# bebop/poly

Measured on AMD Instinct MI355X. Metric: mash.Sketch k-mers hashed/s, higher is better.
Workload: dtype u32

## Files before the change

### poly_amd/csrc/mash_sketch.hip

```cpp
#include <hip/hip_runtime.h>

#include <algorithm>

#include "common.h"
#include "k1_tauq.h"
#include "host_pipeline.h"
#include "multi_device.h"
#include <memory>
#include <string>
#include <type_traits>
#include <vector>

#ifndef PH_WPE
#define PH_WPE 6
#endif
#ifndef PH_CAPK
#define PH_CAPK 12u
#endif
#ifndef PH_ABL
#define PH_ABL 0
#endif
#ifndef PH_SEL_ATOMIC
#define PH_SEL_ATOMIC 0
#endif
#ifndef PH_BS_WIN
#define PH_BS_WIN 4
#endif
static_assert(PH_BS_WIN == 0 || PH_BS_WIN == 4, "the rank pass takes four slots per thread: its window is four");
#ifndef PH_SLAB_SIG
#define PH_SLAB_SIG 6u
#endif
#ifndef PH_SLAB_CW
#define PH_SLAB_CW 6u
#endif
#ifndef PH_SLAB_CF
#define PH_SLAB_CF 0u
#endif
#ifndef PH_SLAB_WPE
#define PH_SLAB_WPE 8
#endif

namespace polyhip {
namespace k1 {

constexpr int THREADS = 256;
constexpr int WAVES = THREADS / 64;
#ifndef PH_WTW
#define PH_WTW 512
#endif
constexpr int WTW = PH_WTW;
constexpr int TW = WTW * WAVES;
constexpr int GROUPS = WTW / (4 * 64);
constexpr int NB = 2048;
constexpr uint32_t MARK0 = 0xFFFFFFFFu, MARK1 = 0u;
constexpr uint32_t LUT_DW = 256;
constexpr int GBATCH = 32;
constexpr uint32_t WL_POSITIONAL = 0x80000000u;
constexpr uint32_t C1 = 0xcc9e2d51u, C2 = 0x1b873593u;

__device__ __forceinline__ uint32_t rotl32(uint32_t x, int r) { return (x << r) | (x >> (32 - r)); }

__device__ __forceinline__ uint32_t premix(uint32_t k)
{
    k *= C1;
    k = rotl32(k, 15);
    k *= C2;
    return k;
}

__device__ __forceinline__ uint32_t chain(uint32_t h) { return rotl32(h, 13) * 5u + 0xe6546b64u; }

__device__ __forceinline__ uint32_t fmix32(uint32_t h)
{
    h ^= h >> 16;
    h *= 0x85ebca6bu;
    h ^= h >> 13;
    h *= 0xc2b2ae35u;
    h ^= h >> 16;
    return h;
}

__device__ __forceinline__ uint32_t funnel_bytes(uint32_t hi, uint32_t lo, uint32_t sh)
{
    return __builtin_amdgcn_alignbyte(hi, lo, sh);
}

__device__ __forceinline__ uint32_t wave_incl_scan(uint32_t v)
{
    v += (uint32_t)__builtin_amdgcn_update_dpp(0, (int)v, 0x111, 0xF, 0xF, true);
    v += (uint32_t)__builtin_amdgcn_update_dpp(0, (int)v, 0x112, 0xF, 0xF, true);
    v += (uint32_t)__builtin_amdgcn_update_dpp(0, (int)v, 0x114, 0xF, 0xF, true);
    v += (uint32_t)__builtin_amdgcn_update_dpp(0, (int)v, 0x118, 0xF, 0xF, true);
    v += (uint32_t)__builtin_amdgcn_update_dpp(0, (int)v, 0x142, 0xA, 0xF, false);
    v += (uint32_t)__builtin_amdgcn_update_dpp(0, (int)v, 0x143, 0xC, 0xF, false);
    return v;
}

struct Smem {
    uint32_t *seqb;
    uint32_t *P;
    uint32_t *cand;
    uint32_t *binned;
    uint32_t *misc;
    uint32_t *lut;
    uint32_t *bins;
    uint32_t *biglist;
    uint32_t listcap;
};

constexpr uint32_t BIG_BIN = 32;
constexpr uint32_t BIG_LIST_CAP = 512;

template <class Bin, class Emit>
__device__ __attribute__((noinline)) void rank_big_bins(const uint32_t *__restrict__ binned, const Bin *__restrict__ bins,
                                              const uint32_t *__restrict__ biglist, uint32_t nbig, uint32_t s, Emit emit)
{
    const int lane = threadIdx.x & 63, wave = threadIdx.x >> 6;
    const uint64_t below = (1ull << lane) - 1ull;
    for (uint32_t q = wave; q < nbig; q += WAVES) {
        const uint32_t b = biglist[q];
        const uint32_t st = b ? bins[b - 1] : 0u, en = bins[b];
        uint32_t base = st, lastv = 0;
        bool first = true;
        while (base < s && base < en) {
            uint32_t m = 0xFFFFFFFFu;
            bool has = false;
            for (uint32_t x = st + lane; x < en; x += 64) {
                const uint32_t o = binned[x];
                if (first || o > lastv) {
                    m = min(m, o);
                    has = true;
                }
            }
            if (__ballot(has) == 0ull)
                break;
#pragma unroll
            for (int d = 32; d >= 1; d >>= 1)
                m = min(m, (uint32_t)__shfl_xor((int)m, d, 64));
            for (uint32_t x0 = st; x0 < en; x0 += 64) {
                const uint32_t x = x0 + lane;
                const bool eq = x < en && binned[x] == m;
                const uint64_t mask = __ballot(eq);
                const uint32_t pos = base + (uint32_t)__builtin_popcountll(mask & below);
                if (eq && pos < s)
                    emit(pos, m);
                base += (uint32_t)__builtin_popcountll(mask);
            }
            lastv = m;
            first = false;
        }
    }
}

template <class ForEach>
__device__ uint32_t bottom_s(const Smem &sm, uint32_t s, uint32_t tau, uint32_t binned_cap, bool keep_partial,
                             ForEach for_each)
{
    const int tid = threadIdx.x;
    uint32_t *bins = sm.P;
    const int sig = 32 - __builtin_clz(tau | 1u);
    const int shift = sig > 11 ? sig - 11 : 0;
    __syncthreads();

    for (int b = tid; b < NB; b += THREADS)
        bins[b] = 0;
    if (tid == 0)
        sm.misc[8] = 0;
    __syncthreads();
    for_each([&](uint32_t h) {
        if (h <= tau)
            atomicAdd(&bins[h >> shift], 1u);
    });
    __syncthreads();

    {
        uint32_t v[8], sum = 0;
#pragma unroll
        for (int i = 0; i < 8; ++i) {
            v[i] = bins[8 * tid + i];
            sum += v[i];
        }
        uint32_t incl = sum;
#pragma unroll
        for (int d = 1; d < 64; d <<= 1) {
            uint32_t t = __shfl_up(incl, d, 64);
            if ((tid & 63) >= d)
                incl += t;
        }
        if ((tid & 63) == 63)
            sm.misc[4 + (tid >> 6)] = incl;
        __syncthreads();
        uint32_t run = incl - sum;
        for (int w = 0; w < (tid >> 6); ++w)
            run += sm.misc[4 + w];
#pragma unroll
        for (int i = 0; i < 8; ++i) {
            bins[8 * tid + i] = run;
            run += v[i];
            if (v[i] > BIG_BIN) {
                const uint32_t slot = atomicAdd(&sm.misc[8], 1u);
                if (slot < BIG_LIST_CAP)
                    sm.seqb[slot] = (uint32_t)(8 * tid + i);
            }
        }
// ... 178 lines not shown
#pragma unroll
            for (int c = 0; c < 4; ++c)
                h[c] ^= k;
        }
#pragma unroll
        for (int c = 0; c < 4; ++c)
            h[c] = PH_ABL == 3 ? h[c] : fmix32(h[c]);
        emit(4u * (uint32_t)wq, h);
    }
    wave_sync();
}

template <int KS, bool LOCKSTEP, class Before, class EmitFull, class EmitPart>
__device__ __forceinline__ void run_tiles(const Smem &sm, const uint32_t *__restrict__ gdw, uint32_t gsh,
                                          int64_t gbytes, int64_t nwin, uint32_t k, uint32_t n_seq_dw, uint32_t n_P_w,
                                          Before before, EmitFull emit_full, EmitPart emit_part)
{
    const int wave = threadIdx.x >> 6;
    uint32_t *seqb = sm.seqb + wave * n_seq_dw;
    uint32_t *P = sm.P + wave * n_P_w;
    const int64_t stage_bytes = (int64_t)n_seq_dw * 4 + 4;
    auto is_full = [&](int64_t t0) { return (nwin - t0) >= (int64_t)WTW && t0 + stage_bytes <= gbytes; };
    Stager<KS> st;
    const int64_t first = (int64_t)wave * WTW;
    if (first < nwin)
        st.load(gdw, gsh, gbytes, first, n_seq_dw, is_full(first));
    for (int64_t T0 = 0; T0 < nwin; T0 += TW) {
        if (LOCKSTEP)
            before(T0);
        const int64_t t0 = T0 + first;
        if (t0 >= nwin)
            continue;
        const bool full = is_full(t0);
        st.store(seqb, gdw, gsh, gbytes, t0, n_seq_dw, full);
        wave_sync();
        if (t0 + TW < nwin)
            st.load(gdw, gsh, gbytes, t0 + TW, n_seq_dw, is_full(t0 + TW));
        if (full) {
            tile_compute<KS>(seqb, P, sm.lut, k, [&](uint32_t w0, const uint32_t(&h)[4]) { emit_full(t0, w0, h, 4u); });
        } else {
            const uint32_t wl = (uint32_t)((nwin - t0) < (int64_t)WTW ? (nwin - t0) : (int64_t)WTW);
            tile_compute<KS>(seqb, P, sm.lut, k, [&](uint32_t w0, const uint32_t(&h)[4]) {
                emit_part(t0, w0, h, w0 >= wl ? 0u : (wl - w0 < 4u ? wl - w0 : 4u));
            });
        }
    }
}

__device__ __forceinline__ void append4(uint32_t *__restrict__ counter, uint32_t *__restrict__ cand, uint32_t cap,
                                        const uint32_t (&h)[4], uint32_t nvalid, uint32_t tau)
{
    bool a[4];
    uint64_t m[4];
    uint32_t cnt[4], total = 0;
#pragma unroll
    for (int c = 0; c < 4; ++c) {
        a[c] = (PH_ABL == 4 ? h[c] == 12345u : h[c] <= tau) && (uint32_t)c < nvalid;
        m[c] = __ballot(a[c]);
        cnt[c] = (uint32_t)__popcll(m[c]);
        total += cnt[c];
    }
    if (total == 0)
        return;
    uint32_t base = 0;
    if ((threadIdx.x & 63) == 0)
        base = atomicAdd(counter, total);
    base = __builtin_amdgcn_readfirstlane(base);
#pragma unroll
    for (int c = 0; c < 4; ++c) {
        if (a[c]) {
            const uint32_t idx = base + __builtin_amdgcn_mbcnt_hi((uint32_t)(m[c] >> 32),
                                                                  __builtin_amdgcn_mbcnt_lo((uint32_t)m[c], 0u));
            if (idx < cap)
                cand[idx] = h[c];
        }
        base += cnt[c];
    }
}

constexpr int BSU = 4;
constexpr int BS_R = 7;
constexpr int BS_R0 = 5;
constexpr uint32_t BS_MARGIN = (PH_BS_WIN + 3u) & ~3u;
static_assert(BS_MARGIN % 4u == 0 && LUT_DW % 4u == 0, "the rank pass reads binned by 16 bytes: binned[0] is 16-byte aligned");
#define BS_SYNC()              \
    do {                       \
        if (PH_ABL != 21)      \
            __syncthreads();   \
    } while (0)
typedef __attribute__((address_space(3))) uint32_t lds_u32;
__device__ __forceinline__ uint32_t lds_addr(const uint32_t *p)
{
    return (uint32_t)(uintptr_t)(const __attribute__((address_space(3))) uint32_t *)p;
}
__device__ __forceinline__ void lds_store4_masked(const uint32_t (&addr)[4], const uint32_t (&v)[4], const uint64_t (&mask)[4])
{
    uint64_t saved;
    asm volatile("s_mov_b64 %0, exec\n\t"
                 "s_mov_b64 exec, %9\n\t"
                 "ds_write_b32 %1, %5\n\t"
                 "s_mov_b64 exec, %10\n\t"
                 "ds_write_b32 %2, %6\n\t"
                 "s_mov_b64 exec, %11\n\t"
                 "ds_write_b32 %3, %7\n\t"
                 "s_mov_b64 exec, %12\n\t"
                 "ds_write_b32 %4, %8\n\t"
                 "s_mov_b64 exec, %0"
                 : "=&s"(saved)
                 : "v"(addr[0]), "v"(addr[1]), "v"(addr[2]), "v"(addr[3]), "v"(v[0]), "v"(v[1]), "v"(v[2]), "v"(v[3]),
                   "s"(mask[0]), "s"(mask[1]), "s"(mask[2]), "s"(mask[3])
                 : "memory");
}
__device__ __forceinline__ void lds_store_masked(uint32_t addr, uint32_t v, uint64_t mask)
{
    uint64_t saved;
    asm volatile("s_mov_b64 %0, exec\n\t"
                 "s_mov_b64 exec, %3\n\t"
                 "ds_write_b32 %1, %2\n\t"
                 "s_mov_b64 exec, %0"
                 : "=&s"(saved)
                 : "v"(addr), "v"(v), "s"(mask)
                 : "memory");
}

template <bool FIN, int BINS_AT = -1>
__device__ void bottom_s_fast(const Smem &sm, uint32_t s, uint32_t tau, uint32_t C, uint32_t nbf_log2,
                              uint32_t *__restrict__ outp, const uint32_t *__restrict__ src, uint32_t first,
                              uint32_t step, uint32_t cnt)
{
    const int tid = threadIdx.x;
    uint32_t tid_o = (uint32_t)tid;
    asm volatile("" : "+v"(tid_o));
    auto fin = [](uint32_t h) { return FIN ? h ^ (h >> 16) : h; };
    uint32_t *bins = sm.bins;
    const uint16_t *bins16 = reinterpret_cast<const uint16_t *>(bins);
    const int sig = 32 - __builtin_clz(tau | 1u);
    const int shift = sig > (int)nbf_log2 ? sig - (int)nbf_log2 : 0;
    auto one = [](uint32_t b) { return 1u << ((b & 1u) << 4); };
    const bool wide = nbf_log2 == 11u;
    uint32_t z;
    asm volatile("v_mov_b32 %0, 0" : "=v"(z));
    if (wide)
        reinterpret_cast<uint4 *>(bins)[tid_o] = make_uint4(z, z, z, z);
    else
        reinterpret_cast<uint2 *>(bins)[tid_o] = make_uint2(z, z);
    if (tid == 0)
        sm.misc[8] = 0;
    if (PH_BS_WIN) {
        if (tid < PH_BS_WIN)
            sm.binned[-1 - (int)tid_o] = 0u;
        else if (tid < 2 * PH_BS_WIN)
            sm.binned[C + tid_o - PH_BS_WIN] = 0xFFFFFFFFu;
    }
    const uint32_t ntrip = (cnt + step - 1u) / step;
    const bool regs = ntrip <= (uint32_t)BS_R && shift >= 1;
    const bool more = ntrip > (uint32_t)BS_R0;
    const uint32_t bins_at = BINS_AT >= 0 ? (uint32_t)BINS_AT : lds_addr(bins);
    uint32_t hr[BS_R], bin_at[BS_R], bin_inc[BS_R];
    uint32_t first_o = first;
    asm volatile("" : "+v"(first_o));
    auto reg_valid = [&](int u) { return first_o < (cnt > (uint32_t)u * step ? cnt - (uint32_t)u * step : 0u); };
    const uint32_t src_at = lds_addr(src) + 4u * first_o, last_at = lds_addr(src) + 4u * ((cnt ? cnt : 1u) - 1u);
    auto reg_load = [&](int u) {
        hr[u] = fin(*reinterpret_cast<const lds_u32 *>((uintptr_t)min(src_at + 4u * (uint32_t)u * step, last_at)));
    };
    auto reg_count = [&](int u) {
        const uint32_t a = hr[u] >> (shift - 1);
        const bool there = reg_valid(u);
        bin_at[u] = there ? a & ~3u : 4u * first_o;
        bin_inc[u] = there ? 1u << ((a & 2u) << 3) : 0u;
        asm volatile("" : "+v"(bin_at[u]), "+v"(bin_inc[u]));
        __hip_atomic_fetch_add(reinterpret_cast<lds_u32 *>((uintptr_t)(bin_at[u] + bins_at)), bin_inc[u], __ATOMIC_RELAXED,
                               __HIP_MEMORY_SCOPE_WORKGROUP);
    };
    if (regs) {
#pragma unroll
        for (int u = 0; u < BS_R0; ++u)
            reg_load(u);
#pragma unroll
        for (int u = BS_R0; u < BS_R; ++u)
            hr[u] = z;
        if (more) {
#pragma unroll
            for (int u = BS_R0; u < BS_R; ++u)
                reg_load(u);
        }
    }
    BS_SYNC();
    if (regs) {
#pragma unroll
        for (int u = 0; u < BS_R0; ++u)
            reg_count(u);
        if (more) {
#pragma unroll
            for (int u = BS_R0; u < BS_R; ++u)
                reg_count(u);
        }
    } else {
        for (uint32_t i0 = first; i0 < cnt; i0 += BSU * step) {
            uint32_t h[BSU];
#pragma unroll
            for (int u = 0; u < BSU; ++u)
                h[u] = i0 + u * step < cnt ? fin(src[i0 + u * step]) : 0u;
#pragma unroll
            for (int u = 0; u < BSU; ++u)
                if (i0 + u * step < cnt) {
                    const uint32_t b = h[u] >> shift;
                    atomicAdd(&bins[b >> 1], one(b));
                }
        }
    }
    BS_SYNC();
    {
        uint32_t w[4];
        if (wide) {
            const uint4 t = reinterpret_cast<const uint4 *>(bins)[tid_o];
            w[0] = t.x, w[1] = t.y, w[2] = t.z, w[3] = t.w;
        } else {
            const uint2 t = reinterpret_cast<const uint2 *>(bins)[tid_o];
            w[0] = t.x, w[1] = t.y, w[2] = 0u, w[3] = 0u;
        }
        uint32_t c[8], sum = 0;
#pragma unroll
        for (int i = 0; i < 8; ++i) {
            c[i] = (w[i >> 1] >> (16 * (i & 1))) & 0xFFFFu;
            sum += c[i];
        }
        const uint32_t incl = wave_incl_scan(sum);
        if ((tid & 63) == 63)
            sm.misc[4 + (tid >> 6)] = incl;
        BS_SYNC();
        uint32_t run = incl - sum;
        for (int w8 = 0; w8 < (tid >> 6); ++w8)
            run += sm.misc[4 + w8];
        const uint32_t b0 = tid_o << (wide ? 3 : 2);
#pragma unroll
        for (int i = 0; i < 4; ++i) {
            w[i] = run | ((run + c[2 * i]) << 16);
            run += c[2 * i] + c[2 * i + 1];
        }
        if (wide)
            reinterpret_cast<uint4 *>(bins)[tid_o] = make_uint4(w[0], w[1], w[2], w[3]);
        else
            reinterpret_cast<uint2 *>(bins)[tid_o] = make_uint2(w[0], w[1]);
        if (max(max(max(c[0], c[1]), max(c[2], c[3])), max(max(c[4], c[5]), max(c[6], c[7]))) > BIG_BIN) {
#pragma unroll
            for (int i = 0; i < 8; ++i)
                if (c[i] > BIG_BIN) {
                    const uint32_t slot = atomicAdd(&sm.misc[8], 1u);
                    if (slot < sm.listcap)
                        sm.biglist[slot] = b0 + (uint32_t)i;
                }
        }
    }
    BS_SYNC();
    if (regs) {
        uint32_t ret[BS_R];
        const uint32_t binned_at = __builtin_amdgcn_readfirstlane(lds_addr(sm.binned));
        auto reg_add = [&](int u) {
            ret[u] = __hip_atomic_fetch_add(reinterpret_cast<lds_u32 *>((uintptr_t)(bin_at[u] + bins_at)), bin_inc[u], __ATOMIC_RELAXED,
                                            __HIP_MEMORY_SCOPE_WORKGROUP);
        };
        auto reg_put = [&](int u) {
            const uint32_t at = __builtin_amdgcn_ubfe(ret[u], bin_inc[u] >> 12, 16u);
            lds_store_masked(binned_at + 4u * at, hr[u], __ballot(bin_inc[u] != 0u));
        };
#pragma unroll
        for (int u = 0; u < BS_R0; ++u)
            reg_add(u);
        if (more) {
#pragma unroll
            for (int u = BS_R0; u < BS_R; ++u)
                reg_add(u);
        }
#pragma unroll
        for (int u = 0; u < BS_R0; ++u)
            reg_put(u);
        if (more) {
#pragma unroll
            for (int u = BS_R0; u < BS_R; ++u)
                reg_put(u);
        }
        asm volatile("s_waitcnt lgkmcnt(0)" ::: "memory");
    } else {
        for (uint32_t i0 = first; i0 < cnt; i0 += BSU * step) {
            uint32_t h[BSU], at[BSU];
#pragma unroll
            for (int u = 0; u < BSU; ++u)
                h[u] = i0 + u * step < cnt ? fin(src[i0 + u * step]) : 0u;
#pragma unroll
            for (int u = 0; u < BSU; ++u)
                if (i0 + u * step < cnt) {
                    const uint32_t b = h[u] >> shift;
                    at[u] = (atomicAdd(&bins[b >> 1], one(b)) >> ((b & 1u) << 4)) & 0xFFFFu;
                }
#pragma unroll
            for (int u = 0; u < BSU; ++u)
                if (i0 + u * step < cnt)
                    sm.binned[at[u]] = h[u];
        }
    }
    BS_SYNC();
    const uint32_t nbig = sm.misc[8];
    const bool by_waves = nbig <= sm.listcap;
    auto rank_in_bin = [&](uint32_t j, uint32_t hv) {
        const uint32_t b = hv >> shift;
        const uint32_t start = b ? bins16[b - 1] : 0u, end = bins16[b];
        if (start >= s || (by_waves && end - start > BIG_BIN))
            return;
        uint32_t pos = start;
        for (uint32_t x = start; x < end; ++x) {
            const uint32_t o = sm.binned[x];
            pos += (o < hv) || (o == hv && x < j);
        }
        if (pos < s)
            outp[pos] = hv;
    };
    const uint32_t e_star = bins16[sm.binned[s - 1] >> shift];
#if PH_BS_WIN
    if (PH_ABL != 22) {
        const uint32_t lim = 1u << shift;
        auto put = [&](uint32_t pos, uint32_t hv) {
            *reinterpret_cast<uint32_t *>(reinterpret_cast<uint8_t *>(outp) + (pos << 2)) = hv;
        };
        for (uint32_t j = 4u * tid_o; j < e_star; j += 4u * THREADS) {
            const uint4 *__restrict__ w4 = reinterpret_cast<const uint4 *>(sm.binned + j);
            const uint4 q0 = w4[-1], q1 = w4[0], q2 = w4[1];
            const uint32_t v[12] = {q0.x, q0.y, q0.z, q0.w, q1.x, q1.y, q1.z, q1.w, q2.x, q2.y, q2.z, q2.w};
            const uint32_t n = e_star - j;
            uint32_t pos[4] = {j, j + 1u, j + 2u, j + 3u};
            bool far[4];
#pragma unroll
            for (int q = 0; q < 4; ++q) {
                const uint32_t hv = v[4 + q];
#pragma unroll
                for (int d = 0; d < 4; ++d) {
                    if (d > q - 1)
                        pos[q] -= v[3 + q - d] > hv ? 1u : 0u;
                    if (d > 2 - q)
                        pos[q] += v[5 + q + d] < hv ? 1u : 0u;
                }
                far[q] = ((v[q] ^ hv) < lim) | ((v[8 + q] ^ hv) < lim);
            }
#pragma unroll
            for (int a = 0; a < 4; ++a)
#pragma unroll
                for (int b = a + 1; b < 4; ++b) {
                    const uint32_t gt = v[4 + a] > v[4 + b] ? 1u : 0u;
                    pos[a] += gt;
                    pos[b] -= gt;
                }
#pragma unroll
            for (int q = 0; q < 4; ++q) {
                if (__builtin_expect(far[q], 0)) {
                    if ((uint32_t)q < n)
                        rank_in_bin(j + (uint32_t)q, v[4 + q]);
                } else if (pos[q] < s && (uint32_t)q < n) {
                    put(pos[q], v[4 + q]);
                }
            }
        }
    }
#else
    for (uint32_t j = tid; j < e_star; j += THREADS)
        rank_in_bin(j, sm.binned[j]);
#endif
    if (by_waves && nbig)
        rank_big_bins(sm.binned, bins16, sm.biglist, nbig, s, [outp](uint32_t pos, uint32_t hv) { outp[pos] = hv; });
}

struct ReadView {
    const uint32_t *gdw;
    uint32_t gsh;
    int64_t gbytes, nwin;
};

__device__ __forceinline__ ReadView view(const uint8_t *__restrict__ seqs, const uint64_t *__restrict__ offs,
                                         uint64_t r, uint32_t k)
{
    ReadView v;
    const uint64_t o0 = offs[r], o1 = offs[r + 1];
    const int64_t n = (int64_t)(o1 - o0);
    v.nwin = n - (int64_t)k;
    v.gsh = (uint32_t)((uintptr_t)(seqs + o0) & 3);
    v.gdw = reinterpret_cast<const uint32_t *>(seqs + o0 - v.gsh);
    v.gbytes = n + v.gsh;
    return v;
}

template <int KS>
__global__ __launch_bounds__(THREADS) __attribute__((amdgpu_waves_per_eu(PH_WPE, 8))) void sketch_fast_kernel(const uint8_t *__restrict__ seqs,
                                                             const uint64_t *__restrict__ offs, uint64_t nseq,
                                                             uint32_t k_rt, uint32_t s, uint32_t *__restrict__ out,
                                                             uint32_t n_seq_dw, uint32_t n_P_w, uint32_t n_P,
                                                             uint32_t capf, uint32_t nbf_log2)
{
    extern __shared__ __attribute__((aligned(16))) uint32_t smem_raw[];
    Smem sm;
    sm.seqb = smem_raw;
    sm.P = sm.seqb + WAVES * n_seq_dw;
    sm.cand = sm.P + n_P;
    sm.binned = sm.cand + capf + BS_MARGIN;
    sm.misc = sm.binned + capf + BS_MARGIN;
    sm.lut = sm.misc + 16;
    sm.bins = sm.P;
    sm.biglist = sm.seqb;
    sm.listcap = BIG_LIST_CAP;

    const uint32_t k = KS > 0 ? (uint32_t)KS : k_rt;
    const int tid = threadIdx.x;
    sm.lut[tid] = premix((uint32_t)tid) ^ k;
    auto nothing = [](int64_t) {};

    for (uint64_t r = blockIdx.x; r < nseq; r += gridDim.x) {
        const ReadView rv = view(seqs, offs, r, k);
        if (rv.nwin <= 0)
            continue;
        uint32_t *__restrict__ outp = out + r * (uint64_t)s;

        if (rv.nwin < (int64_t)s) {
            __syncthreads();
            auto put = [&](int64_t t0, uint32_t w0, const uint32_t(&h)[4], uint32_t nvalid) {
#pragma unroll
                for (int c = 0; c < 4; ++c)
                    if ((uint32_t)c < nvalid)
                        outp[t0 + w0 + c] = h[c];
            };
            run_tiles<KS, false>(sm, rv.gdw, rv.gsh, rv.gbytes, rv.nwin, k, n_seq_dw, n_P_w, nothing, put, put);
            continue;
        }

        uint32_t tau0 = 0xFFFFFFFFu;
        {
            const uint64_t target = (uint64_t)s + 6ull * (uint64_t)__builtin_sqrtf((float)s) + 16ull;
            if ((int64_t)target < rv.nwin)
                tau0 = (uint32_t)((target << 32) / (uint64_t)rv.nwin);
        }
        bool ok = tau0 != 0xFFFFFFFFu || rv.nwin <= (int64_t)capf;
        __syncthreads();
        if (tid == 0)
            sm.misc[0] = 0;
        __syncthreads();
        uint32_t C = 0;
        if (ok) {
            auto keep = [&](int64_t, uint32_t, const uint32_t(&h)[4], uint32_t nvalid) {
                append4(&sm.misc[0], sm.cand, capf, h, nvalid, tau0);
            };
            run_tiles<KS, false>(sm, rv.gdw, rv.gsh, rv.gbytes, rv.nwin, k, n_seq_dw, n_P_w, nothing, keep, keep);
            __syncthreads();
            C = sm.misc[0];
            ok = C >= s && C <= capf;
        }
        if (ok) {
            if (PH_ABL == 5) {
                for (uint32_t i = tid; i < s; i += THREADS)
                    outp[i] = sm.cand[i];
            } else {
                bottom_s_fast<false>(sm, s, tau0, C, nbf_log2, outp, sm.cand, (uint32_t)tid, THREADS, C);
            }
        } else if (tid == 0) {
            outp[0] = MARK0;
            outp[1] = MARK1;
        }
    }
}

template <int KS> struct Slabs {
    static constexpr int NBLK = KS >> 2, TAIL = KS & 3;
    static constexpr int DUPD = NBLK + 2;
    const uint32_t *__restrict__ gdw;
    uint32_t gsh;
    uint32_t *__restrict__ seqb;
    uint32_t *__restrict__ P;
    const uint32_t *__restrict__ lut;
    int lane;

    uint32_t u_inside;
    uint32_t gb32;
    template <bool SH> __device__ __forceinline__ void gload_inside(uint32_t u, uint32_t &lo, uint32_t &hi) const
    {
        const uint32_t *__restrict__ slab = gdw + (uint64_t)u * 64;
        uint32_t off = (uint32_t)lane * 4u;
        asm volatile("" : "+v"(off));
        const uint8_t *__restrict__ p = reinterpret_cast<const uint8_t *>(slab) + off;
        lo = *reinterpret_cast<const uint32_t *>(p);
        hi = SH ? *reinterpret_cast<const uint32_t *>(p + 4) : 0u;
    }
    __device__ __forceinline__ void gload(uint32_t u, uint32_t &lo, uint32_t &hi) const
    {
        const uint32_t *__restrict__ slab = gdw + (uint64_t)u * 64;
// ... 151 lines not shown
    S.u_inside = rv.gbytes >= 65 * 4 ? (uint32_t)(((rv.gbytes >> 2) - 65) >> 6) + 1u : 0u;
    S.gb32 = (uint32_t)rv.gbytes;
    const uint32_t nfull = (uint32_t)(rv.nwin >> 8), rem = (uint32_t)rv.nwin & 255u;
    uint32_t cnt = 0;
#if PH_SEL_ATOMIC
    capw -= 1u;
    if (S.lane == 0)
        seg[capw] = 0u;
#endif
    if (a >= b)
        return cnt;
    uint32_t l1, h1;
    S.gload(a, l1, h1);
    if (a & 1) {
        S.template stage<1>(l1, h1);
        wave_sync();
        S.gload(a + 1, l1, h1);
        S.template premix_unit<1>();
    } else {
        S.template stage<0>(l1, h1);
        wave_sync();
        S.gload(a + 1, l1, h1);
        S.template premix_unit<0>();
    }
    auto step = [&](auto par, auto main, auto sh, uint32_t i) {
        constexpr int P = decltype(par)::value;
        constexpr bool MAIN = decltype(main)::value, SH = decltype(sh)::value;
        uint32_t h[4];
        S.template stage<1 - P, SH>(l1, h1);
        wave_sync();
        if (MAIN)
            S.template gload_inside<SH>(i + 2, l1, h1);
        else
            S.gload(i + 2, l1, h1);
        if (PH_ABL != 15)
            S.template premix_unit<1 - P>();
        wave_sync();
        S.template hash<P>(h);
        if (PH_ABL == 11) {
            if ((h[0] ^ h[1] ^ h[2] ^ h[3]) == 0x12345u)
                seg[0] = h[0];
        } else if (MAIN || __builtin_expect(i < nfull, 1)) {
            append_own<false>(seg, capw, cnt, h, 4u, tauq);
        } else {
            const int mine = (int)rem - 4 * S.lane;
            append_own<true>(seg, capw, cnt, h, mine <= 0 ? 0u : (mine < 4 ? (uint32_t)mine : 4u), tauq);
        }
        wave_sync();
    };
    using P0 = std::integral_constant<int, 0>;
    using P1 = std::integral_constant<int, 1>;
    using T = std::true_type;
    using F = std::false_type;
    const uint32_t lim = nfull < b ? nfull : b;
    const uint32_t ins = S.u_inside >= 2u ? S.u_inside - 2u : 0u;
    const uint32_t m = ins < lim ? ins : lim;
    uint32_t i = a;
    auto main_loop = [&](auto sh) {
        if ((i & 1) && i < m)
            step(P1{}, T{}, sh, i++);
        for (; i + 1 < m; i += 2) {
            step(P0{}, T{}, sh, i);
            step(P1{}, T{}, sh, i + 1);
        }
        if (i < m)
            step(P0{}, T{}, sh, i++);
    };
    if (S.gsh)
        main_loop(T{});
    else
        main_loop(F{});
    for (; i < b; ++i) {
        if (i & 1)
            step(P1{}, F{}, T{}, i);
        else
            step(P0{}, F{}, T{}, i);
    }
    return cnt;
}

template <int KS>
__global__ __launch_bounds__(THREADS) __attribute__((amdgpu_waves_per_eu(PH_SLAB_WPE, 8))) void sketch_slab_kernel(
    const uint8_t *__restrict__ seqs, const uint64_t *__restrict__ offs, uint64_t nseq, uint32_t s, uint32_t *__restrict__ out,
    uint32_t n_seq_dw, uint32_t n_P_w, uint32_t n_span, uint32_t capw, uint32_t capf, uint32_t nbf_log2)
{
    extern __shared__ __attribute__((aligned(16))) uint32_t smem_raw[];
    Smem sm;
    sm.lut = smem_raw;
    sm.seqb = smem_raw + LUT_DW;
    sm.P = sm.seqb + WAVES * n_seq_dw;
    sm.bins = sm.seqb;
    sm.binned = sm.bins + ((1u << nbf_log2) >> 1) + BS_MARGIN;
    sm.biglist = sm.binned + capf + BS_MARGIN;
    sm.listcap = (uint32_t)(sm.seqb + n_span - sm.biglist);
    sm.misc = sm.seqb + n_span;
    sm.cand = sm.misc + 16;
    constexpr uint32_t k = (uint32_t)KS;
    const int tid = threadIdx.x, wave = __builtin_amdgcn_readfirstlane(tid >> 6);
    sm.lut[tid] = premix((uint32_t)tid) ^ k;
    uint32_t *seg = sm.cand + wave * capw;

    for (uint64_t r = blockIdx.x; r < nseq; r += gridDim.x) {
        const ReadView rv = view(seqs, offs, r, k);
        if (rv.nwin <= 0)
            continue;
        uint32_t *__restrict__ outp = out + r * (uint64_t)s;
        if (rv.nwin < (int64_t)s)
            continue;
        const uint32_t tauq = slab_tauq(s + PH_SLAB_SIG * (uint32_t)__builtin_sqrtf((float)s) + 16u, rv.nwin);
        __syncthreads();
        const uint32_t cw = PH_ABL == 14 ? tauq >> 31 : run_slabs<KS>(sm, rv, n_seq_dw, n_P_w, seg, capw, tauq);
        if ((tid & 63) == 0)
            sm.misc[10 + wave] = cw;
        __syncthreads();
        if (PH_ABL == 11 || PH_ABL == 12 || PH_ABL == 14) {
            if (sm.misc[10] + sm.misc[11] + sm.misc[12] + sm.misc[13] == 0xFFFFFFF0u)
                outp[0] = cw;
            continue;
        }
        const uint32_t c0 = sm.misc[10], c1 = sm.misc[11], c2 = sm.misc[12], c3 = sm.misc[13];
        const uint32_t C = c0 + c1 + c2 + c3;
        const bool ok = max(max(c0, c1), max(c2, c3)) <= capw - (PH_SEL_ATOMIC ? 1u : 0u) && C >= s && C <= capf;
        if (ok)
            bottom_s_fast<true, (int)(LUT_DW * 4u)>(sm, s, tauq, C, nbf_log2, outp, seg, (uint32_t)(tid & 63), 64u, cw);
        else if (tid == 0) {
            outp[0] = MARK0;
            outp[1] = MARK1;
        }
    }
}

template <int KS>
__global__ __launch_bounds__(THREADS) void sketch_general_kernel(const uint8_t *__restrict__ seqs,
                                                                const uint64_t *__restrict__ offs, uint32_t k_rt,
                                                                uint32_t s, uint32_t *__restrict__ out,
                                                                uint32_t n_seq_dw, uint32_t n_P_w, uint32_t n_P,
                                                                uint32_t cap, uint64_t nseq, int take_positional)
{
    extern __shared__ __attribute__((aligned(16))) uint32_t smem_raw[];
    Smem sm;
    sm.seqb = smem_raw;
    sm.P = sm.seqb + WAVES * n_seq_dw;
    sm.cand = sm.P + n_P;
    sm.binned = sm.cand + cap;
    sm.misc = sm.binned + cap;
    sm.lut = sm.misc + 16;
    __shared__ uint32_t wl[GBATCH];
    __shared__ uint32_t nwl;

    const uint32_t k = KS > 0 ? (uint32_t)KS : k_rt;
    const int tid = threadIdx.x;
    sm.lut[tid] = premix((uint32_t)tid) ^ k;

    for (uint64_t base = (uint64_t)blockIdx.x * GBATCH; base < nseq; base += (uint64_t)gridDim.x * GBATCH) {
        __syncthreads();
        if (tid == 0)
            nwl = 0;
        __syncthreads();
        {
            const uint64_t r = base + tid;
            if (tid < GBATCH && r < nseq) {
                const int64_t nwin = (int64_t)(offs[r + 1] - offs[r]) - (int64_t)k;
                uint32_t need = 0;
                if (nwin >= (int64_t)s) {
                    const uint32_t *row = out + r * (uint64_t)s;
                    if (row[0] == MARK0 && row[1] == MARK1)
                        need = 1;
                } else if (nwin > 0 && take_positional) {
                    need = 2;
                }
                if (need)
                    wl[atomicAdd(&nwl, 1u)] = (uint32_t)tid | (need == 2 ? WL_POSITIONAL : 0u);
            }
        }
        __syncthreads();
        const uint32_t nredo = nwl;
    for (uint32_t q = 0; q < nredo; ++q) {
        const uint32_t entry = wl[q];
        const uint64_t r = base + (entry & ~WL_POSITIONAL);
        const ReadView rv = view(seqs, offs, r, k);
        uint32_t *__restrict__ outp = out + r * (uint64_t)s;
        __syncthreads();
        if (entry & WL_POSITIONAL) {
            auto put = [&](int64_t t0, uint32_t w0, const uint32_t(&h)[4], uint32_t nvalid) {
#pragma unroll
                for (int c = 0; c < 4; ++c)
                    if ((uint32_t)c < nvalid)
                        outp[t0 + w0 + c] = h[c];
            };
            run_tiles<KS, false>(sm, rv.gdw, rv.gsh, rv.gbytes, rv.nwin, k, n_seq_dw, n_P_w, [](int64_t) {}, put, put);
            continue;
        }
        if (tid == 0) {
            sm.misc[0] = 0;
            sm.misc[1] = 0xFFFFFFFFu;
        }
        __syncthreads();
        auto shrink_shared = [&]() {
            const uint32_t C = sm.misc[0];
            bottom_s(sm, s, sm.misc[1], cap, true, [&](auto f) {
                for (uint32_t i = tid; i < C; i += THREADS)
                    f(sm.cand[i]);
            });
        };
        auto append = [&](int64_t, uint32_t, const uint32_t(&h)[4], uint32_t nvalid) {
            append4(&sm.misc[0], sm.cand, cap, h, nvalid, sm.misc[1]);
        };
// ... 89 lines not shown
#pragma unroll
            for (int c = 0; c < 4; ++c) {
                const int64_t w = base + c * THREADS + tid;
                if (w < nwin) {
                    const uint32_t h = murmur3_window(sp + w, k);
                    if (h <= tau)
                        sm.cand[atomicAdd(&misc[0], 1u)] = h;
                }
            }
        }
        __syncthreads();
        shrink();
        for (uint32_t i = tid; i < s; i += THREADS)
            outp[i] = sm.cand[i];
    }
}

__global__ __launch_bounds__(THREADS) void sketch_tiny_kernel(const uint8_t *__restrict__ seqs,
                                                             const uint64_t *__restrict__ offs, uint64_t nseq, uint32_t k,
                                                             uint32_t s, uint32_t *__restrict__ out,
                                                             unsigned long long *__restrict__ first_panic)
{
    const int tid = threadIdx.x;
    for (uint64_t r = blockIdx.x; r < nseq; r += gridDim.x) {
        const uint64_t o0 = offs[r];
        const int64_t nwin = (int64_t)(offs[r + 1] - o0) - (int64_t)k;
        if (nwin <= 0)
            continue;
        if (s == 0) {
            if (tid == 0)
                atomicMin(first_panic, (unsigned long long)r);
            continue;
        }
        const uint8_t *__restrict__ sp = seqs + o0;
        const uint32_t h0 = murmur3_window(sp, k);
        bool under = false;
        for (int64_t w = 1 + tid; w < nwin && !under; w += THREADS)
            under = murmur3_window(sp + w, k) < h0;
        if (__syncthreads_or(under ? 1 : 0)) {
            if (tid == 0)
                atomicMin(first_panic, (unsigned long long)r);
        } else if (tid == 0) {
            out[r] = h0;
        }
    }
}

struct Launch {
    uint32_t n_seq_dw, n_P_w, n_P, n_P_fast, nbf_log2, nbf_log2_slab, capf, cap, capw, capf_slab, n_span;
    size_t smem_fast, smem_general, smem_slab;
};

static Launch plan(uint32_t k, uint32_t s)
{
    Launch L;
    const uint32_t nblk = k / 4;
    L.n_seq_dw = ((WTW / 4 + nblk + 2) + 3u) & ~3u;
    L.n_P_w = WTW + 4 * nblk;
    L.n_P = WAVES * L.n_P_w;
    L.n_P_fast = L.n_P < 1024u ? 1024u : L.n_P;
    L.nbf_log2 = L.n_P_fast >= 2048u ? 11u : 10u;
    if (L.n_P < (uint32_t)NB)
        L.n_P = NB;
    const uint32_t s4 = (s + 3u) & ~3u;
    uint32_t rt = 1;
    while ((uint64_t)rt * rt < s)
        ++rt;
    L.capf = (s4 + PH_CAPK * rt + 64u + 63u) & ~63u;
    L.cap = s4 + TW + 64u;
    const size_t common = (size_t)WAVES * L.n_seq_dw + L.n_P + 16 + 256;
    L.smem_fast = ((size_t)WAVES * L.n_seq_dw + L.n_P_fast + 16 + 256 + 2 * (size_t)L.capf + 2 * BS_MARGIN) * 4;
    if (PH_ABL == 7)
        L.smem_fast = 70 * 1024;
    L.smem_general = (common + 2 * (size_t)L.cap) * 4;
    {
        const uint32_t target = s + PH_SLAB_SIG * rt + 16u;
        const uint32_t exp_w = (target + WAVES - 1) / WAVES;
        uint32_t rw = 1;
        while ((uint64_t)rw * rw < exp_w)
            ++rw;
        L.capw = (exp_w + PH_SLAB_CW * rw + 8u + 63u) & ~63u;
        L.capf_slab = PH_SLAB_CF ? ((target + PH_SLAB_CF * rt + 8u + 63u) & ~63u) : L.capf;
    }
    L.nbf_log2_slab = 11;
    {
        const uint32_t rings = WAVES * (L.n_seq_dw + L.n_P_w);
        const uint32_t sorted = ((1u << L.nbf_log2_slab) >> 1) + L.capf_slab + 2 * BS_MARGIN + L.capf_slab / (BIG_BIN + 1) + 1;
        L.n_span = rings > sorted ? rings : sorted;
    }
    L.smem_slab = ((size_t)LUT_DW + L.n_span + 16 + (size_t)WAVES * L.capw) * 4;
#ifdef PH_LDS_PAD
    L.smem_slab += PH_LDS_PAD;
#endif
    return L;
}

constexpr uint64_t SLAB_ROUNDS = 32;

static unsigned persistent_grid(size_t smem, uint64_t n, uint64_t rounds = 4)
{
    const uint64_t per_cu = std::max<uint64_t>(1, std::min<uint64_t>(8, (160 * 1024) / std::max<size_t>(smem, 1)));
    return (unsigned)std::min<uint64_t>(n, 256 * per_cu * rounds);
}

template <int KS>
static int launch(const uint8_t *d_seqs, const uint64_t *d_offs, uint64_t n, uint32_t k, uint32_t s,
                  uint32_t *d_out, const Launch &L, hipStream_t st)
{
    PH_REQUIRE(L.capf % 4u == 0 && L.capf_slab % 4u == 0 && (WAVES * L.n_seq_dw + L.n_P_fast + L.capf + BS_MARGIN) % 4u == 0 &&
                   (LUT_DW + ((1u << L.nbf_log2_slab) >> 1) + BS_MARGIN) % 4u == 0,
               "polyhip_mash_sketch_batch: the sorted buffer of the LDS layout is not 16-byte aligned");
    auto general = sketch_general_kernel<KS>;
    PH_HIP(hipFuncSetAttribute(reinterpret_cast<const void *>(general), hipFuncAttributeMaxDynamicSharedMemorySize,
                               (int)L.smem_general));
    bool slabs = false;
    if constexpr (KS > 0) {
        slabs = !env_is("POLYHIP_K1_SLABS", '0') && L.smem_slab <= 64 * 1024 && s < 32768u;
        if (slabs) {
            auto slab = sketch_slab_kernel<KS>;
            PH_HIP(hipFuncSetAttribute(reinterpret_cast<const void *>(slab), hipFuncAttributeMaxDynamicSharedMemorySize,
                                       (int)L.smem_slab));
            hipLaunchKernelGGL(slab, dim3(persistent_grid(L.smem_slab, n, SLAB_ROUNDS)), dim3(THREADS), L.smem_slab, st, d_seqs, d_offs, n, s,
                               d_out, L.n_seq_dw, L.n_P_w, L.n_span, L.capw, L.capf_slab, L.nbf_log2_slab);
        }
    }
    if (!slabs) {
        auto fast = sketch_fast_kernel<KS>;
        PH_HIP(hipFuncSetAttribute(reinterpret_cast<const void *>(fast), hipFuncAttributeMaxDynamicSharedMemorySize,
                                   (int)L.smem_fast));
        hipLaunchKernelGGL(fast, dim3(persistent_grid(L.smem_fast, n)), dim3(THREADS), L.smem_fast, st, d_seqs, d_offs, n,
                           k, s, d_out, L.n_seq_dw, L.n_P_w, L.n_P_fast, L.capf, L.nbf_log2);
    }
    PH_HIP(hipGetLastError());
    const unsigned ggrid = (unsigned)std::min<uint64_t>((n + GBATCH - 1) / GBATCH, persistent_grid(L.smem_general, n));
    hipLaunchKernelGGL(general, dim3(ggrid), dim3(THREADS), L.smem_general, st, d_seqs, d_offs, k, s, d_out, L.n_seq_dw,
                       L.n_P_w, L.n_P, L.cap, n, slabs ? 1 : 0);
    PH_HIP(hipGetLastError());
    return POLYHIP_OK;
}

}
}

using namespace polyhip;

extern "C" {

int polyhip_mash_sketch_batch_dev(const uint8_t *d_seqs, const uint64_t *d_offsets, uint64_t n, uint32_t k,
                                  uint32_t s, uint32_t *d_out, polyhip_stream_t stream)
{
    if (n == 0)
        return POLYHIP_OK;
    PH_REQUIRE(d_seqs && d_offsets && (d_out || s == 0), "polyhip_mash_sketch_batch: null pointer");
    PH_REQUIRE(s <= (1u << 24), "polyhip_mash_sketch_batch: SketchSize %u > 2^24 is not implemented", s);
    hipStream_t st = as_stream(stream);
    if (s < 2) {
        unsigned long long *d_first = nullptr, h_first = ~0ull;
        PH_HIP(hipMallocAsync(reinterpret_cast<void **>(&d_first), sizeof h_first, st));
        StreamFree guard{d_first, st};
        PH_HIP(hipMemsetAsync(d_first, 0xFF, sizeof h_first, st));
        hipLaunchKernelGGL(k1::sketch_tiny_kernel, dim3((unsigned)std::min<uint64_t>(n, 4096)), dim3(k1::THREADS), 0, st, d_seqs,
                           d_offsets, n, k, s, d_out, d_first);
        PH_HIP(hipGetLastError());
        PH_HIP(hipMemcpyAsync(&h_first, d_first, sizeof h_first, hipMemcpyDeviceToHost, st));
        PH_HIP(guard.release());
        PH_HIP(hipStreamSynchronize(st));
        if (h_first != ~0ull)
            return set_error(POLYHIP_ERR_PANIC,
                             "mash.Sketch with SketchSize %u indexes Sketches[-1] on sequence %llu (mash.go:%s): the reference panics",
                             s, h_first + (unsigned long long)md::base().item, s == 0 ? "96" : "98");
        return POLYHIP_OK;
    }
    const k1::Launch L = k1::plan(k <= 4096 ? k : 4096, s <= 8192 ? s : 8192);
    if (s > 8192 || k > 4096 || L.smem_general > 160 * 1024) {
        const uint32_t s4 = (s + 3u) & ~3u;
        const uint32_t cap = 2 * s4 + 2 * k1::WIDE_ROUND;
        const uint64_t per_wg = 2ull * cap * sizeof(uint32_t), budget = 4ull << 30;
        const unsigned grid = (unsigned)std::max<uint64_t>(
            1, std::min<uint64_t>(std::min<uint64_t>(n, s > 16384 ? 256 : 1024), budget / per_wg));
        uint32_t *scratch = nullptr;
        PH_HIP(hipMallocAsync(reinterpret_cast<void **>(&scratch), (size_t)grid * per_wg, st));
        StreamFree guard{scratch, st};
        hipLaunchKernelGGL(k1::sketch_wide_kernel, dim3(grid), dim3(k1::THREADS), 0, st, d_seqs, d_offsets, n, k, s, d_out, scratch,
                           cap);
        PH_HIP(hipGetLastError());
        PH_HIP(guard.release());
        return POLYHIP_OK;
    }
    const uint64_t CHUNK = 1ull << 30;
    for (uint64_t i0 = 0; i0 < n; i0 += CHUNK) {
        const uint64_t m = n - i0 < CHUNK ? n - i0 : CHUNK;
        const uint64_t *offs = d_offsets + i0;
        uint32_t *outp = d_out + i0 * (uint64_t)s;
        int rc;
        switch (k) {
        case 17: rc = k1::launch<17>(d_seqs, offs, m, k, s, outp, L, st); break;
        case 21: rc = k1::launch<21>(d_seqs, offs, m, k, s, outp, L, st); break;
        case 31: rc = k1::launch<31>(d_seqs, offs, m, k, s, outp, L, st); break;
        default: rc = k1::launch<0>(d_seqs, offs, m, k, s, outp, L, st); break;
        }
        if (rc != POLYHIP_OK)
            return rc;
    }
    return POLYHIP_OK;
}

// ... 157 lines not shown
```

Measured before the change: 999.1 billion.

## Pack bin-count scan, flag big bins via SWAR, add wave-level small-bin ranking

Reworks the bottom-s selection: the per-thread bin-count scan now works on packed 16-bit pairs with SWAR adds and perm instead of unpacking eight counters. Big bins are detected with a packed overflow test and stored as a 16-bit list (doubling list capacity). rank_big_bins makes its bin bounds wave-uniform and handles bins of at most 64 entries with a readlane comparison loop, and the per-element in-bin ranking moves into a separate noinline function. The slab kernel's bin count becomes a compile-time constant. This adds a 15-bit count limit, enforced by a new host check, plus extra code paths that could raise register pressure.

After: 1002 billion (median of 6 runs). Within noise of the previous version (+0.3%).

```diff
diff --git a/poly_amd/csrc/mash_sketch.hip b/poly_amd/csrc/mash_sketch.hip
--- a/poly_amd/csrc/mash_sketch.hip
+++ b/poly_amd/csrc/mash_sketch.hip
@@ -27,6 +27,12 @@
 #define PH_BS_WIN 4
 #endif
 static_assert(PH_BS_WIN == 0 || PH_BS_WIN == 4, "the rank pass takes four slots per thread: its window is four");
+#ifndef PH_BS_LIST_WIN
+#define PH_BS_LIST_WIN 0
+#endif
+#ifndef PH_BS_SCAN_PACKED
+#define PH_BS_SCAN_PACKED 1
+#endif
 #ifndef PH_SLAB_SIG
 #define PH_SLAB_SIG 6u
 #endif
@@ -111,15 +117,30 @@
 constexpr uint32_t BIG_BIN = 32;
 constexpr uint32_t BIG_LIST_CAP = 512;
 
-template <class Bin, class Emit>
+template <class Bin, class List, class Emit>
 __device__ __attribute__((noinline)) void rank_big_bins(const uint32_t *__restrict__ binned, const Bin *__restrict__ bins,
-                                              const uint32_t *__restrict__ biglist, uint32_t nbig, uint32_t s, Emit emit)
-{
-    const int lane = threadIdx.x & 63, wave = threadIdx.x >> 6;
+                                              const List *__restrict__ biglist, uint32_t nbig, uint32_t s, Emit emit)
+{
+    const int lane = threadIdx.x & 63, wave = __builtin_amdgcn_readfirstlane(threadIdx.x >> 6);
     const uint64_t below = (1ull << lane) - 1ull;
     for (uint32_t q = wave; q < nbig; q += WAVES) {
-        const uint32_t b = biglist[q];
-        const uint32_t st = b ? bins[b - 1] : 0u, en = bins[b];
+        const uint32_t b = __builtin_amdgcn_readfirstlane((uint32_t)biglist[q]);
+        const uint32_t st = b ? __builtin_amdgcn_readfirstlane((uint32_t)bins[b - 1]) : 0u;
+        const uint32_t en = __builtin_amdgcn_readfirstlane((uint32_t)bins[b]);
+        if (st >= s || en <= st)
+            continue;
+        if (en - st <= 64u) {
+            const uint32_t n = en - st;
+            const uint32_t mine = binned[st + min((uint32_t)lane, n - 1u)];
+            uint32_t pos = st;
+            for (uint32_t i = 0; i < n; ++i) {
+                const uint32_t o = (uint32_t)__builtin_amdgcn_readlane((int)mine, (int)i);
+                pos += (o < mine || (o == mine && i < (uint32_t)lane)) ? 1u : 0u;
+            }
+            if ((uint32_t)lane < n && pos < s)
+                emit(pos, mine);
+            continue;
+        }
         uint32_t base = st, lastv = 0;
         bool first = true;
         while (base < s && base < en) {
@@ -464,6 +485,8 @@
 constexpr int BS_R = 7;
 constexpr int BS_R0 = 5;
 constexpr uint32_t BS_MARGIN = (PH_BS_WIN + 3u) & ~3u;
+constexpr uint32_t NBF_LOG2_SLAB = 11;
+constexpr uint32_t BS_LIST_OVER = PH_BS_WIN && PH_BS_LIST_WIN ? (uint32_t)PH_BS_WIN : BIG_BIN;
 static_assert(BS_MARGIN % 4u == 0 && LUT_DW % 4u == 0, "the rank pass reads binned by 16 bytes: binned[0] is 16-byte aligned");
 #define BS_SYNC()              \
     do {                       \
@@ -505,14 +528,35 @@
                  : "memory");
 }
 
-template <bool FIN, int BINS_AT = -1>
-__device__ void bottom_s_fast(const Smem &sm, uint32_t s, uint32_t tau, uint32_t C, uint32_t nbf_log2,
+__device__ __attribute__((noinline)) void rank_whole_bins(const uint32_t *__restrict__ binned, const uint16_t *__restrict__ bins16,
+                                                          int shift, uint32_t s, uint32_t e_star, uint32_t skip_over,
+                                                          uint32_t *__restrict__ outp)
+{
+    for (uint32_t j = threadIdx.x; j < e_star; j += THREADS) {
+        const uint32_t hv = binned[j];
+        const uint32_t b = hv >> shift;
+        const uint32_t start = b ? bins16[b - 1] : 0u, end = bins16[b];
+        if (start >= s || end - start > skip_over)
+            continue;
+        uint32_t pos = start;
+        for (uint32_t x = start; x < end; ++x) {
+            const uint32_t o = binned[x];
+            pos += (o < hv) || (o == hv && x < j);
+        }
+        if (pos < s)
+            outp[pos] = hv;
+    }
+}
+
+template <bool FIN, int BINS_AT = -1, int NBF_LOG2 = 0>
+__device__ void bottom_s_fast(const Smem &sm, uint32_t s, uint32_t tau, uint32_t C, uint32_t nbf_log2_rt,
                               uint32_t *__restrict__ outp, const uint32_t *__restrict__ src, uint32_t first,
                               uint32_t step, uint32_t cnt)
 {
     const int tid = threadIdx.x;
     uint32_t tid_o = (uint32_t)tid;
     asm volatile("" : "+v"(tid_o));
+    const uint32_t nbf_log2 = NBF_LOG2 > 0 ? (uint32_t)NBF_LOG2 : nbf_log2_rt;
     auto fin = [](uint32_t h) { return FIN ? h ^ (h >> 16) : h; };
     uint32_t *bins = sm.bins;
     const uint16_t *bins16 = reinterpret_cast<const uint16_t *>(bins);
@@ -526,12 +570,12 @@
         reinterpret_cast<uint4 *>(bins)[tid_o] = make_uint4(z, z, z, z);
     else
         reinterpret_cast<uint2 *>(bins)[tid_o] = make_uint2(z, z);
-    if (tid == 0)
+    if (tid_o == 0u)
         sm.misc[8] = 0;
     if (PH_BS_WIN) {
-        if (tid < PH_BS_WIN)
+        if (tid_o < (uint32_t)PH_BS_WIN)
             sm.binned[-1 - (int)tid_o] = 0u;
-        else if (tid < 2 * PH_BS_WIN)
+        else if (tid_o < 2u * (uint32_t)PH_BS_WIN)
             sm.binned[C + tid_o - PH_BS_WIN] = 0xFFFFFFFFu;
     }
     const uint32_t ntrip = (cnt + step - 1u) / step;
@@ -602,38 +646,75 @@
             const uint2 t = reinterpret_cast<const uint2 *>(bins)[tid_o];
             w[0] = t.x, w[1] = t.y, w[2] = 0u, w[3] = 0u;
         }
-        uint32_t c[8], sum = 0;
+        const uint32_t b0 = tid_o << (wide ? 3 : 2);
+        constexpr uint32_t OVER = (0x7FFFu - BS_LIST_OVER) * 0x10001u;
+        const uint32_t f01 = ((w[0] + OVER) & 0x80008000u) | (((w[1] + OVER) & 0x80008000u) >> 1);
+        const uint32_t f23 = ((w[2] + OVER) & 0x80008000u) | (((w[3] + OVER) & 0x80008000u) >> 1);
+        const uint32_t flags = f01 | (f23 >> 2);
+        uint32_t run, sum;
+#if PH_BS_SCAN_PACKED
+        const uint32_t t = (w[0] + w[1]) + (w[2] + w[3]);
+        sum = (t & 0xFFFFu) + (t >> 16);
+#else
+        uint32_t c[8];
+        sum = 0;
 #pragma unroll
         for (int i = 0; i < 8; ++i) {
             c[i] = (w[i >> 1] >> (16 * (i & 1))) & 0xFFFFu;
             sum += c[i];
         }
+#endif
         const uint32_t incl = wave_incl_scan(sum);
-        if ((tid & 63) == 63)
-            sm.misc[4 + (tid >> 6)] = incl;
+        if ((tid_o & 63u) == 63u)
+            sm.misc[4 + (tid_o >> 6)] = incl;
+        if (__ballot(flags != 0u) != 0ull) {
+            const uint32_t nl = (uint32_t)__builtin_popcount(flags);
+            uint32_t slot = nl ? atomicAdd(&sm.misc[8], nl) : 0u;
+            uint16_t *list = reinterpret_cast<uint16_t *>(sm.biglist);
+#pragma unroll
+            for (int i = 0; i < 8; ++i)
+                if (flags & (1u << (16 * (i & 1) + 15 - (i >> 1)))) {
+                    if (slot < sm.listcap)
+                        list[slot] = (uint16_t)(b0 + (uint32_t)i);
+                    ++slot;
+                }
+        }
+        if (PH_BS_LIST_WIN && sig == 32 && tid_o == (uint32_t)(THREADS - 1)) {
+            const uint32_t top = (wide ? w[3] : w[1]) >> 16;
+            if (top != 0u && top <= BS_LIST_OVER) {
+                const uint32_t slot = atomicAdd(&sm.misc[8], 1u);
+                if (slot < sm.listcap)
+                    reinterpret_cast<uint16_t *>(sm.biglist)[slot] = (uint16_t)((1u << nbf_log2) - 1u);
+            }
+        }
         BS_SYNC();
-        uint32_t run = incl - sum;
-        for (int w8 = 0; w8 < (tid >> 6); ++w8)
+        run = incl - sum;
+#if PH_BS_SCAN_PACKED
+        {
+            const uint4 tot = *reinterpret_cast<const uint4 *>(sm.misc + 4);
+            const uint32_t wv = __builtin_amdgcn_readfirstlane(tid_o >> 6);
+            run += (tot.x & (wv > 0u ? ~0u : 0u)) + (tot.y & (wv > 1u ? ~0u : 0u)) + (tot.z & (wv > 2u ? ~0u : 0u));
+        }
+        uint32_t both = run | (run << 16);
+#pragma unroll
+        for (int i = 0; i < 4; ++i) {
+            const uint32_t cnts = w[i];
+            w[i] = both + (cnts << 16);
+            both = __builtin_amdgcn_perm(0u, w[i] + cnts, 0x03020302u);
+        }
+#else
+        for (int w8 = 0; w8 < (int)(tid_o >> 6); ++w8)
             run += sm.misc[4 + w8];
-        const uint32_t b0 = tid_o << (wide ? 3 : 2);
 #pragma unroll
         for (int i = 0; i < 4; ++i) {
             w[i] = run | ((run + c[2 * i]) << 16);
             run += c[2 * i] + c[2 * i + 1];
         }
+#endif
         if (wide)
             reinterpret_cast<uint4 *>(bins)[tid_o] = make_uint4(w[0], w[1], w[2], w[3]);
         else
             reinterpret_cast<uint2 *>(bins)[tid_o] = make_uint2(w[0], w[1]);
-        if (max(max(max(c[0], c[1]), max(c[2], c[3])), max(max(c[4], c[5]), max(c[6], c[7]))) > BIG_BIN) {
-#pragma unroll
-            for (int i = 0; i < 8; ++i)
-                if (c[i] > BIG_BIN) {
-                    const uint32_t slot = atomicAdd(&sm.misc[8], 1u);
-                    if (slot < sm.listcap)
-                        sm.biglist[slot] = b0 + (uint32_t)i;
-                }
-        }
     }
     BS_SYNC();
     if (regs) {
@@ -685,6 +766,7 @@
     BS_SYNC();
     const uint32_t nbig = sm.misc[8];
     const bool by_waves = nbig <= sm.listcap;
+#if !PH_BS_LIST_WIN
     auto rank_in_bin = [&](uint32_t j, uint32_t hv) {
         const uint32_t b = hv >> shift;
         const uint32_t start = b ? bins16[b - 1] : 0u, end = bins16[b];
@@ -698,6 +780,7 @@
         if (pos < s)
             outp[pos] = hv;
     };
+#endif
     const uint32_t e_star = bins16[sm.binned[s - 1] >> shift];
 #if PH_BS_WIN
     if (PH_ABL != 22) {
@@ -722,7 +805,7 @@
                     if (d > 2 - q)
                         pos[q] += v[5 + q + d] < hv ? 1u : 0u;
                 }
-                far[q] = ((v[q] ^ hv) < lim) | ((v[8 + q] ^ hv) < lim);
+                far[q] = (((v[q] ^ hv) < lim) & (j != 0u)) | ((v[8 + q] ^ hv) < lim);
             }
 #pragma unroll
             for (int a = 0; a < 4; ++a)
@@ -734,21 +817,31 @@
                 }
 #pragma unroll
             for (int q = 0; q < 4; ++q) {
+#if !PH_BS_LIST_WIN
                 if (__builtin_expect(far[q], 0)) {
                     if ((uint32_t)q < n)
                         rank_in_bin(j + (uint32_t)q, v[4 + q]);
-                } else if (pos[q] < s && (uint32_t)q < n) {
+                    continue;
+                }
+#endif
+                if (!far[q] && pos[q] < s && (uint32_t)q < n)
                     put(pos[q], v[4 + q]);
-                }
-            }
-        }
-    }
+            }
+        }
+    }
+    if (nbig == 0u)
+        return;
+    if (by_waves || !PH_BS_LIST_WIN)
+        rank_big_bins(sm.binned, bins16, reinterpret_cast<const uint16_t *>(sm.biglist), by_waves ? nbig : 0u, s,
+                      [outp](uint32_t pos, uint32_t hv) { outp[pos] = hv; });
+    else
+        rank_whole_bins(sm.binned, bins16, shift, s, e_star, 0xFFFFFFFFu, outp);
 #else
-    for (uint32_t j = tid; j < e_star; j += THREADS)
-        rank_in_bin(j, sm.binned[j]);
-#endif
+    rank_whole_bins(sm.binned, bins16, shift, s, e_star, by_waves ? BIG_BIN : 0xFFFFFFFFu, outp);
     if (by_waves && nbig)
-        rank_big_bins(sm.binned, bins16, sm.biglist, nbig, s, [outp](uint32_t pos, uint32_t hv) { outp[pos] = hv; });
+        rank_big_bins(sm.binned, bins16, reinterpret_cast<const uint16_t *>(sm.biglist), nbig, s,
+                      [outp](uint32_t pos, uint32_t hv) { outp[pos] = hv; });
+#endif
 }
 
 struct ReadView {
@@ -787,7 +880,7 @@
     sm.lut = sm.misc + 16;
     sm.bins = sm.P;
     sm.biglist = sm.seqb;
-    sm.listcap = BIG_LIST_CAP;
+    sm.listcap = 2u * BIG_LIST_CAP;
 
     const uint32_t k = KS > 0 ? (uint32_t)KS : k_rt;
     const int tid = threadIdx.x;
@@ -1105,7 +1198,7 @@
 template <int KS>
 __global__ __launch_bounds__(THREADS) __attribute__((amdgpu_waves_per_eu(PH_SLAB_WPE, 8))) void sketch_slab_kernel(
     const uint8_t *__restrict__ seqs, const uint64_t *__restrict__ offs, uint64_t nseq, uint32_t s, uint32_t *__restrict__ out,
-    uint32_t n_seq_dw, uint32_t n_P_w, uint32_t n_span, uint32_t capw, uint32_t capf, uint32_t nbf_log2)
+    uint32_t n_seq_dw, uint32_t n_P_w, uint32_t n_span, uint32_t capw, uint32_t capf)
 {
     extern __shared__ __attribute__((aligned(16))) uint32_t smem_raw[];
     Smem sm;
@@ -1113,15 +1206,17 @@
     sm.seqb = smem_raw + LUT_DW;
     sm.P = sm.seqb + WAVES * n_seq_dw;
     sm.bins = sm.seqb;
-    sm.binned = sm.bins + ((1u << nbf_log2) >> 1) + BS_MARGIN;
+    sm.binned = sm.bins + ((1u << NBF_LOG2_SLAB) >> 1) + BS_MARGIN;
     sm.biglist = sm.binned + capf + BS_MARGIN;
-    sm.listcap = (uint32_t)(sm.seqb + n_span - sm.biglist);
+    sm.listcap = 2u * (uint32_t)(sm.seqb + n_span - sm.biglist);
     sm.misc = sm.seqb + n_span;
     sm.cand = sm.misc + 16;
     constexpr uint32_t k = (uint32_t)KS;
     const int tid = threadIdx.x, wave = __builtin_amdgcn_readfirstlane(tid >> 6);
     sm.lut[tid] = premix((uint32_t)tid) ^ k;
     uint32_t *seg = sm.cand + wave * capw;
+    uint32_t capw_s = capw;
+    asm volatile("" : "+s"(capw_s));
 
     for (uint64_t r = blockIdx.x; r < nseq; r += gridDim.x) {
         const ReadView rv = view(seqs, offs, r, k);
@@ -1132,7 +1227,7 @@
             continue;
         const uint32_t tauq = slab_tauq(s + PH_SLAB_SIG * (uint32_t)__builtin_sqrtf((float)s) + 16u, rv.nwin);
         __syncthreads();
-        const uint32_t cw = PH_ABL == 14 ? tauq >> 31 : run_slabs<KS>(sm, rv, n_seq_dw, n_P_w, seg, capw, tauq);
+        const uint32_t cw = PH_ABL == 14 ? tauq >> 31 : run_slabs<KS>(sm, rv, n_seq_dw, n_P_w, seg, capw_s, tauq);
         if ((tid & 63) == 0)
             sm.misc[10 + wave] = cw;
         __syncthreads();
@@ -1145,7 +1240,7 @@
         const uint32_t C = c0 + c1 + c2 + c3;
         const bool ok = max(max(c0, c1), max(c2, c3)) <= capw - (PH_SEL_ATOMIC ? 1u : 0u) && C >= s && C <= capf;
         if (ok)
-            bottom_s_fast<true, (int)(LUT_DW * 4u)>(sm, s, tauq, C, nbf_log2, outp, seg, (uint32_t)(tid & 63), 64u, cw);
+            bottom_s_fast<true, (int)(LUT_DW * 4u), (int)NBF_LOG2_SLAB>(sm, s, tauq, C, NBF_LOG2_SLAB, outp, seg, (uint32_t)(tid & 63), 64u, cw);
         else if (tid == 0) {
             outp[0] = MARK0;
             outp[1] = MARK1;
@@ -1401,11 +1496,11 @@
         L.capw = (exp_w + PH_SLAB_CW * rw + 8u + 63u) & ~63u;
         L.capf_slab = PH_SLAB_CF ? ((target + PH_SLAB_CF * rt + 8u + 63u) & ~63u) : L.capf;
     }
-    L.nbf_log2_slab = 11;
+    L.nbf_log2_slab = NBF_LOG2_SLAB;
     {
         const uint32_t rings = WAVES * (L.n_seq_dw + L.n_P_w);
-        const uint32_t sorted = ((1u << L.nbf_log2_slab) >> 1) + L.capf_slab + 2 * BS_MARGIN + L.capf_slab / (BIG_BIN + 1) + 1;
-        L.n_span = rings > sorted ? rings : sorted;
+        const uint32_t sorted = ((1u << L.nbf_log2_slab) >> 1) + L.capf_slab + 2 * BS_MARGIN + (L.capf_slab / (BS_LIST_OVER + 1) + 2) / 2;
+        L.n_span = ((rings > sorted ? rings : sorted) + 3u) & ~3u;
     }
     L.smem_slab = ((size_t)LUT_DW + L.n_span + 16 + (size_t)WAVES * L.capw) * 4;
 #ifdef PH_LDS_PAD
@@ -1427,8 +1522,10 @@
                   uint32_t *d_out, const Launch &L, hipStream_t st)
 {
     PH_REQUIRE(L.capf % 4u == 0 && L.capf_slab % 4u == 0 && (WAVES * L.n_seq_dw + L.n_P_fast + L.capf + BS_MARGIN) % 4u == 0 &&
-                   (LUT_DW + ((1u << L.nbf_log2_slab) >> 1) + BS_MARGIN) % 4u == 0,
+                   (LUT_DW + ((1u << L.nbf_log2_slab) >> 1) + BS_MARGIN) % 4u == 0 && L.n_span % 4u == 0,
                "polyhip_mash_sketch_batch: the sorted buffer of the LDS layout is not 16-byte aligned");
+    PH_REQUIRE(L.capf < 32768u - BS_LIST_OVER && L.capf_slab < 32768u - BS_LIST_OVER,
+               "polyhip_mash_sketch_batch: the fast pass's candidate buffer does not fit 15-bit counts");
     auto general = sketch_general_kernel<KS>;
     PH_HIP(hipFuncSetAttribute(reinterpret_cast<const void *>(general), hipFuncAttributeMaxDynamicSharedMemorySize,
                                (int)L.smem_general));
@@ -1440,7 +1537,7 @@
             PH_HIP(hipFuncSetAttribute(reinterpret_cast<const void *>(slab), hipFuncAttributeMaxDynamicSharedMemorySize,
                                        (int)L.smem_slab));
             hipLaunchKernelGGL(slab, dim3(persistent_grid(L.smem_slab, n, SLAB_ROUNDS)), dim3(THREADS), L.smem_slab, st, d_seqs, d_offs, n, s,
-                               d_out, L.n_seq_dw, L.n_P_w, L.n_span, L.capw, L.capf_slab, L.nbf_log2_slab);
+                               d_out, L.n_seq_dw, L.n_P_w, L.n_span, L.capw, L.capf_slab);
         }
     }
     if (!slabs) {
```
